# tlk00/BitMagic

Measured on NVIDIA B200. Metric: aggregator input 64Kbit-blocks/s, higher is better.
Workload: dtype u32

## Files before the change

### bitmagic_b200/capi.py

```python
from __future__ import annotations

import ctypes as C
import os
from pathlib import Path

import numpy as np

_HERE = Path(__file__).resolve().parent
LIB_PATH = Path(os.environ.get("BMB200_LIB", str(_HERE / "libbmb200.so")))

OK = 0
ERR_BADALLOC, ERR_BADARG, ERR_RANGE, ERR_RS_IDX_MISSING = 1, 2, 3, 7
ERR_CUDA, ERR_NODEVICE, ERR_UNSUPPORTED = 200, 201, 202
BLOCK_WORDS, BLOCK_BYTES, BLOCK_BITS = 2048, 8192, 65536
GAP_MAX_WORDS, GAP_THRESHOLD, GAP_UNIT_WORDS, SUPERBLOCK = 1280, 1276, 8, 256
BLK_NULL, BLK_FULL, BLK_BIT, BLK_GAP = 0, 1, 2, 3
OP_OR, OP_AND, OP_AND_SUB, OP_XOR, OP_SHIFT_R_AND = 0, 1, 2, 3, 4
F_COUNT_ONLY, F_OPT_NONE, F_OPT_COMPRESS, F_OR_TARGET = 1, 0, 2, 4

SYMBOLS = [
    "bmb200_init", "bmb200_destroy", "bmb200_error_msg", "bmb200_last_error", "bmb200_ctx_set_stream",
    "bmb200_ctx_get_stream", "bmb200_ctx_sync", "bmb200_ctx_launch_count", "bmb200_device_info", "bmb200_ctx_set_tuning",
    "bmb200_set_upload", "bmb200_set_upload_vectors", "bmb200_set_adopt_device", "bmb200_set_info",
    "bmb200_set_column_sizes", "bmb200_set_download", "bmb200_set_device_ptrs", "bmb200_set_free",
    "bmb200_synth_set", "bmb200_aggregate", "bmb200_result_optimize", "bmb200_result_total",
    "bmb200_result_fetch_meta", "bmb200_result_sizes", "bmb200_result_fetch", "bmb200_result_device_ptrs",
    "bmb200_result_free", "bmb200_aggregate_host", "bmb200_rs_build", "bmb200_rs_export", "bmb200_rs_total",
    "bmb200_rank_batch", "bmb200_select_batch", "bmb200_rank_batch_dev", "bmb200_select_batch_dev",
    "bmb200_rs_free", "bmb200_rs_rebuild", "bmb200_aggregate_batch", "bmb200_result_group_totals", "bmb200_result_or_target",
    "bmb200_scan", "bmb200_set_upload_blobs", "bmb200_result_fetch_view", "bmb200_ctx_bind_host_numa",
    "bmb200_shard_range", "bmb200_comm_unique_id", "bmb200_comm_init", "bmb200_comm_info", "bmb200_comm_destroy",
    "bmb200_exchange_popcounts", "bmb200_exchange_fence", "bmb200_exchange_fetch", "bmb200_ctx_trim", "bmb200_binop",
    "bmb200_set_upload_slabs", "bmb200_host_slabs_prefetch", "bmb200_host_slab_alloc", "bmb200_host_slab_free",
    "bmb200_result_fetch_view_async", "bmb200_result_fetch_wait", "bmb200_exchange_mode",
    "bmb200_result_fetch_column",
]
OP_SUB = 5
COMM_ID_BYTES = 128
TUNE_GAP_MODE, TUNE_CTAS_PER_SM, TUNE_HOST_THREADS = 0, 1, 2


class PackedSetC(C.Structure):
    _fields_ = [
        ("n_vec", C.c_uint32), ("n_blocks", C.c_uint32),
        ("desc", C.c_void_p), ("bit_base", C.c_void_p), ("gap_base", C.c_void_p),
        ("bit_pool", C.c_void_p), ("gap_pool", C.c_void_p),
    ]


class VecBlocksC(C.Structure):
    _fields_ = [("n_blocks", C.c_uint32), ("kind", C.c_void_p), ("ptr", C.c_void_p)]


class HostSlabC(C.Structure):
# ... 109 lines not shown
            pass

    def sync(self):
        self.check(lib().bmb200_ctx_sync(self._h), "ctx_sync")

    def set_stream(self, cuda_stream: int):
        self.check(lib().bmb200_ctx_set_stream(self._h, C.c_void_p(int(cuda_stream))), "ctx_set_stream")

    def get_stream(self) -> int:
        s = C.c_void_p(0)
        self.check(lib().bmb200_ctx_get_stream(self._h, C.byref(s)), "ctx_get_stream")
        return int(s.value or 0)

    def set_tuning(self, key: int, value: int):
        self.check(lib().bmb200_ctx_set_tuning(self._h, int(key), int(value)), "ctx_set_tuning")

    def launch_count(self) -> int:
        n = C.c_uint64(0)
        self.check(lib().bmb200_ctx_launch_count(self._h, C.byref(n)), "launch_count")
        return int(n.value)

    def trim(self):
        self.check(lib().bmb200_ctx_trim(self._h), "ctx_trim")

    def bind_host_numa(self) -> int:
        node = C.c_int(-1)
        self.check(lib().bmb200_ctx_bind_host_numa(self._h, C.byref(node)), "ctx_bind_host_numa")
        return node.value

    @staticmethod
# ... 383 lines not shown
```

### bitmagic_b200/csrc/agg_kernel.cuh

```cuda
#pragma once
#include "common.cuh"
#include <type_traits>

namespace bmb200 {

constexpr int kAggThreads = 512;
constexpr int kAggWarps   = kAggThreads / 32;
constexpr int kAggChunk   = 1024;
#ifndef BMB200_AGG_CHUNK_WIDE
#define BMB200_AGG_CHUNK_WIDE 1408
#endif
constexpr int kAggChunkWide = BMB200_AGG_CHUNK_WIDE;

#ifndef BMB200_CTAS_PER_SM
#define BMB200_CTAS_PER_SM 2
#endif
#ifndef BMB200_GAP_STAGES
#define BMB200_GAP_STAGES (BMB200_CTAS_PER_SM >= 3 ? 3 : 4)
#endif
#ifndef BMB200_BIT_UNROLL
#define BMB200_BIT_UNROLL 4
#endif
#ifndef BMB200_GAP_CHUNK
#define BMB200_GAP_CHUNK 16384
#endif
#ifndef BMB200_LANES_PER_BLOCK
#define BMB200_LANES_PER_BLOCK 16
#endif
#ifndef BMB200_VAR_UNROLL2
#define BMB200_VAR_UNROLL2 1
#endif
#ifndef BMB200_VAR_SLEEP_NS
#define BMB200_VAR_SLEEP_NS 64
#endif
constexpr uint32_t kLanesPerBlock = BMB200_LANES_PER_BLOCK;
constexpr uint32_t kGroupsPerWarp = 32u / kLanesPerBlock;
constexpr int      kGapStages     = BMB200_GAP_STAGES;
constexpr uint32_t kGapChunkBytes = BMB200_GAP_CHUNK;
constexpr uint32_t kRingBytes     = kGapStages * kGapChunkBytes;
constexpr int      kCtasPerSm     = BMB200_CTAS_PER_SM;
constexpr int      kBitUnroll     = BMB200_BIT_UNROLL;
constexpr uint32_t kRingWords     = kRingBytes / 4;
constexpr uint32_t kGapMaxBytes   = 2560;
constexpr int      kMaxChunks     = (kAggChunk * 4096) / (int)kGapChunkBytes + 4;
constexpr uint32_t kRingTail      = kGapMaxBytes + 512;
constexpr size_t   kAggRingSmem   = kRingBytes + kRingTail;
constexpr uint32_t kLiveAlign     = 8192u;
__host__ inline size_t agg_dyn_smem(size_t static_bytes, size_t reserved_bytes)
{
// ... 21 lines not shown
    uint32_t  compress;
    uint32_t  store_blocks;
    uint32_t  gap_mode;
    uint32_t  dyn_bytes;
    uint32_t  binary;
    uint64_t  gap_pool_bytes;
    uint32_t* blocks;
    uint32_t* popcnt;
    uint64_t* digest;
    uint32_t* nruns;
    uint8_t*  kind;
    uint16_t* gaps;
    unsigned long long* total;
    uint32_t* or_blocks;
    uint32_t* work_counter;
};

constexpr uint32_t kFlNull0 = 1u;
constexpr uint32_t kFlFull0 = 2u;
constexpr uint32_t kFlFull1 = 4u;
constexpr uint32_t kRelMask = BMB200_DESC_REL_MASK;
constexpr uint32_t kEntFlat = BMB200_DESC_GAP_FLAT >> 2;
constexpr uint32_t kFlatMinBlocks = 16u;

__device__ __forceinline__ uint32_t smem_u32(const void* p) { return (uint32_t)__cvta_generic_to_shared(p); }
__device__ __forceinline__ void mbar_init(uint64_t* bar, uint32_t count)
{
    asm volatile("mbarrier.init.shared::cta.b64 [%0], %1;" :: "r"(smem_u32(bar)), "r"(count) : "memory");
}
__device__ __forceinline__ void mbar_arrive_expect_tx(uint64_t* bar, uint32_t bytes)
// ... 24 lines not shown
}
__device__ __forceinline__ uint32_t atoms_add(uint32_t a, uint32_t v)
{
    uint32_t old; asm volatile("atom.shared.add.u32 %0, [%1], %2;" : "=r"(old) : "r"(a), "r"(v) : "memory"); return old;
}
__device__ __forceinline__ void sts32(uint32_t a, uint32_t v) { asm volatile("st.shared.u32 [%0], %1;" :: "r"(a), "r"(v) : "memory"); }
__device__ __forceinline__ void bulk_g2s(void* smem_dst, const void* gsrc, uint32_t bytes, uint64_t* bar)
{
    asm volatile("cp.async.bulk.shared::cluster.global.mbarrier::complete_tx::bytes [%0], [%1], %2, [%3];"
                 :: "r"(smem_u32(smem_dst)), "l"(gsrc), "r"(bytes), "r"(smem_u32(bar)) : "memory");
}
__device__ __forceinline__ void fence_proxy_async()
{
    asm volatile("fence.proxy.async.shared::cta;" ::: "memory");
}

__device__ __forceinline__ uint32_t lds32(uint32_t a) { uint32_t v; asm volatile("ld.shared.u32 %0, [%1];" : "=r"(v) : "r"(a)); return v; }
__device__ __forceinline__ uint32_t lds16(uint32_t a) { uint16_t v; asm volatile("ld.shared.u16 %0, [%1];" : "=h"(v) : "r"(a)); return (uint32_t)v; }
__device__ __forceinline__ uint4 lds128(uint32_t a)
{
    uint4 v; asm volatile("ld.shared.v4.u32 {%0,%1,%2,%3}, [%4];" : "=r"(v.x), "=r"(v.y), "=r"(v.z), "=r"(v.w) : "r"(a)); return v;
}
__device__ __forceinline__ void reds_and(uint32_t a, uint32_t v) { asm volatile("red.shared.and.b32 [%0], %1;" :: "r"(a), "r"(v) : "memory"); }
__device__ __forceinline__ void reds_xor(uint32_t a, uint32_t v) { asm volatile("red.shared.xor.b32 [%0], %1;" :: "r"(a), "r"(v) : "memory"); }
__device__ __forceinline__ uint32_t bmsk(uint32_t pos, uint32_t width)
{
    uint32_t m; asm("bmsk.clamp.b32 %0, %1, %2;" : "=r"(m) : "r"(pos), "r"(width)); return m;
}

template <int OP>
__device__ __forceinline__ void acc_apply0(uint4& a, const uint4& v)
{
    if (OP == BMB200_OP_OR)       { a.x |= v.x; a.y |= v.y; a.z |= v.z; a.w |= v.w; }
    else if (OP == BMB200_OP_XOR) { a.x ^= v.x; a.y ^= v.y; a.z ^= v.z; a.w ^= v.w; }
    else                          { a.x &= v.x; a.y &= v.y; a.z &= v.z; a.w &= v.w; }
}
__device__ __forceinline__ void acc_or(uint4& a, const uint4& v)
{
    a.x |= v.x; a.y |= v.y; a.z |= v.z; a.w |= v.w;
}

template <int OP, bool ROLE1>
__device__ __forceinline__ void bit_phase(const uint4* __restrict__ seg, const uint32_t* lst, uint32_t n, uint4& acc)
{
    const uint4 ident = (!ROLE1 && (OP == BMB200_OP_AND || OP == BMB200_OP_AND_SUB))
                            ? make_uint4(~0u, ~0u, ~0u, ~0u) : make_uint4(0u, 0u, 0u, 0u);
    for (uint32_t i = 0; i < n; i += kBitUnroll) {
        uint4 v[kBitUnroll];
#pragma unroll
        for (int u = 0; u < kBitUnroll; ++u) {
            if (i + u < n) v[u] = ld_stream_v4(seg + (size_t)lst[i + u] * (kBlockWords / 4));
            else           v[u] = ident;
        }
#pragma unroll
        for (int u = 0; u < kBitUnroll; ++u) {
            if (ROLE1) acc_or(acc, v[u]); else acc_apply0<OP>(acc, v[u]);
        }
    }
}

template <bool XOR>
__device__ __forceinline__ void apply_word(uint32_t a, uint32_t m)
{
    if (XOR) reds_xor(a, m); else reds_and(a, ~m);
}
template <bool XOR>
__device__ __forceinline__ void apply_run(uint32_t Ls, uint32_t s, uint32_t e)
{
    const uint32_t ws = s >> 5, we = e >> 5;
    const uint32_t m0 = 0xffffffffu << (s & 31u);
    const uint32_t m1 = 0xffffffffu >> (31u - (e & 31u));
// ... 273 lines not shown
        if (tid == 0) {
            const uint32_t lvl = runs <= 124u ? 0u : runs <= 252u ? 1u : runs <= 508u ? 2u : 3u;
            gout[runs] = 65535u;
            gout[0] = (uint16_t)((R.x & 1u) | (lvl << 1) | (runs << 3));
        }
    }
    if (tid == 0) {
        p.popcnt[col] = tpc;
        p.digest[col] = dg;
        p.nruns[col]  = runs;
        p.kind[col]   = (uint8_t)kd;
        if (tpc) atomicAdd(p.total + grp, (unsigned long long)tpc);
    }
}

template <int OP>
__global__ void __launch_bounds__(kAggThreads, kCtasPerSm) agg_kernel(const AggParams p)
{
    constexpr int kChunkN = (OP == BMB200_OP_AND_SUB) ? kAggChunk : kAggChunkWide;
    constexpr int kMaxChunksN = (kChunkN * 4096) / (int)kGapChunkBytes + 4;
    extern __shared__ __align__(128) uint8_t dyn_smem[];
    const uint32_t dyn_s = smem_u32(dyn_smem);
    const uint32_t k_off = ((dyn_s + kLiveAlign - 1u) & ~(kLiveAlign - 1u)) - dyn_s;
    if (k_off + kLiveAlign + (uint32_t)kAggRingSmem > p.dyn_bytes) __trap();
    uint32_t* K = reinterpret_cast<uint32_t*>(dyn_smem + k_off);
    uint32_t* ring = reinterpret_cast<uint32_t*>(dyn_smem + k_off + kLiveAlign);

    __shared__ uint32_t lst_bit0[kChunkN];
    __shared__ uint32_t lst_bit1[kChunkN];
    __shared__ uint32_t lst_gap[kChunkN];
    __shared__ uint32_t s_cfirst[kMaxChunksN];
    __shared__ __align__(8) uint64_t s_full[kGapStages];
    __shared__ uint32_t s_done[kGapStages];
    __shared__ __align__(8) uint64_t s_wfull[kAggWarps * kFlatSlots];
    __shared__ uint32_t s_flat_next;
    __shared__ uint2 s_wpk[2][kAggWarps];
    __shared__ uint32_t s_stat[4];
    __shared__ uint32_t s_flat[3];
    __shared__ uint32_t s_col, s_gap_next;
    __shared__ uint32_t s_pc[kAggWarps], s_tr[kAggWarps], s_dg[kAggWarps];

    constexpr bool kIsXor = (OP == BMB200_OP_XOR);
    constexpr bool kIsAnd = (OP == BMB200_OP_AND || OP == BMB200_OP_AND_SUB);
    constexpr int  kFlatList = (OP == BMB200_OP_OR) ? 0 : (OP == BMB200_OP_AND_SUB) ? 1 : -1;

    const int tid = threadIdx.x, lane = tid & 31, warp = tid >> 5;
    const uint32_t M = p.set.n_vec;
    uint4* K4 = reinterpret_cast<uint4*>(K);
    uint32_t Ks, ring_s;
    asm volatile("mov.u32 %0, %1;" : "=r"(Ks) : "r"(smem_u32(K)));
    asm volatile("mov.u32 %0, %1;" : "=r"(ring_s) : "r"(smem_u32(ring)));
    uint32_t done_s, wfull_s, flat_next_s;
    asm volatile("mov.u32 %0, %1;" : "=r"(flat_next_s) : "r"(smem_u32(&s_flat_next)));
    asm volatile("mov.u32 %0, %1;" : "=r"(done_s) : "r"(smem_u32(s_done)));
    asm volatile("mov.u32 %0, %1;" : "=r"(wfull_s) : "r"(smem_u32(&s_wfull[warp * kFlatSlots])));
    uint32_t wphase = 0;
    uint32_t wchunk[kFlatSlots];
    uint32_t gseq = 0;

    if (tid == 0) {
#pragma unroll
        for (int s = 0; s < kGapStages; ++s) mbar_init(&s_full[s], 1u);
#pragma unroll
        for (int w = 0; w < kAggWarps * (int)kFlatSlots; ++w) mbar_init(&s_wfull[w], 1u);
        asm volatile("fence.mbarrier_init.release.cluster;" ::: "memory");
    }
    uint32_t next_item = 0;
    if (tid == 0) next_item = atomicAdd(p.work_counter, 1u);
    __syncthreads();

    for (;;) {
        if (tid == 0) s_col = next_item;
        __syncthreads();
        const uint32_t item = s_col;
        if (item >= p.n_cols * p.n_groups) break;
        if (tid == 0) next_item = atomicAdd(p.work_counter, 1u);
        const uint32_t colx = item / p.n_groups, grp = item - colx * p.n_groups;
        const uint32_t col = grp * p.n_cols + colx;
        const uint32_t nb = p.nb_from + colx;
        const uint32_t gb0 = p.goff[2u * grp], gb1 = p.goff[2u * grp + 1u], gb2 = p.goff[2u * grp + 2u];
        const uint32_t n0 = gb1 - gb0, n1 = (OP == BMB200_OP_AND_SUB) ? gb2 - gb1 : 0u;
        const uint32_t ntot = n0 + n1;
        const uint32_t* gmem = p.group + gb0;
        uint32_t rule = 0u;
        if (p.binary) {
            const uint32_t* dr = p.set.desc + (size_t)nb * M;
            rule = binop_rule(p.binary - 1u, dr[gmem[0]] & 3u, dr[gmem[1]] & 3u);
            if (rule & kRuleMerge) {
                if (p.kind[col] != 0xffu) { __syncthreads(); continue; }
                rule = kRuleComputed;
// ... 35 lines not shown
                const uint32_t lt = (1u << lane) - 1u;
                const uint32_t m0 = __ballot_sync(0xffffffffu, c0), m1 = __ballot_sync(0xffffffffu, c1);
                const uint32_t m2 = __ballot_sync(0xffffffffu, c2), m3 = __ballot_sync(0xffffffffu, c3);
                if (lane == 0) s_wpk[trip][warp] = make_uint2(__popc(m0) | (__popc(m1) << 16), __popc(m2) | (__popc(m3) << 16));
                __syncthreads();
                uint2 x = (lane < kAggWarps) ? s_wpk[trip][lane] : make_uint2(0u, 0u);
#pragma unroll
                for (int o = 1; o < kAggWarps; o <<= 1) {
                    const uint32_t y0 = __shfl_up_sync(0xffffffffu, x.x, o), y1 = __shfl_up_sync(0xffffffffu, x.y, o);
                    if (lane >= o) { x.x += y0; x.y += y1; }
                }
                const uint32_t t01 = __shfl_sync(0xffffffffu, x.x, kAggWarps - 1), t23 = __shfl_sync(0xffffffffu, x.y, kAggWarps - 1);
                uint32_t e01 = __shfl_sync(0xffffffffu, x.x, (warp + 31) & 31), e23 = __shfl_sync(0xffffffffu, x.y, (warp + 31) & 31);
                if (warp == 0) { e01 = 0u; e23 = 0u; }
                e01 += run01; e23 += run23;
                if (c0) lst_bit0[(e01 & 0xffffu) + __popc(m0 & lt)] = rel;
                if (c1) lst_bit1[(e01 >> 16) + __popc(m1 & lt)] = rel;
                if (c2) lst_gap[(e23 & 0xffffu) + __popc(m2 & lt)] = rel;
                if (c3) lst_gap[kChunkN - 1 - ((e23 >> 16) + __popc(m3 & lt))] = rel;
                run01 += t01; run23 += t23;
            }
            fl = __reduce_or_sync(0xffffffffu, fl);
            nfull0 = warp_sum(nfull0);
            nonflat = __reduce_or_sync(0xffffffffu, nonflat);
            if (lane == 0) { if (fl) atomicOr(&s_stat[0], fl); if (nfull0) atomicAdd(&s_stat[3], nfull0); if (nonflat) s_flat[2] = 1u; }
            const uint32_t nbit0 = run01 & 0xffffu, nbit1 = run01 >> 16, ngap0 = run23 & 0xffffu, ngap1 = run23 >> 16;
            if (tid == 0) { s_stat[1] += nbit0; s_stat[2] += ngap0; }
            __syncthreads();

            const uint32_t want0 = kIsAnd ? 0u : 1u;
            bool ok0 = false, ok1 = false;
            bool flat = false;
// ... 44 lines not shown
            auto issue_fill = [&](uint32_t wlo, uint32_t wbytes, uint32_t c, bool mirror) {
                const uint32_t s = (gseq + c) % kGapStages;
                const uint32_t off = c * kGapChunkBytes;
                const uint32_t bytes = min(kGapChunkBytes, wbytes - off);
                const uint32_t extra = (s || !mirror) ? 0u : min(kGapMaxBytes, bytes);
                const uint8_t* src = reinterpret_cast<const uint8_t*>(gseg) + (size_t)wlo * 16u + off;
                mbar_arrive_expect_tx(&s_full[s], bytes + extra);
                bulk_g2s(reinterpret_cast<uint8_t*>(ring) + s * kGapChunkBytes, src, bytes, &s_full[s]);
                if (extra) bulk_g2s(reinterpret_cast<uint8_t*>(ring) + kRingBytes, src, extra, &s_full[s]);
            };
            auto flat_big = [&](uint32_t wbytes) -> bool {
                return BMB200_FLAT_SLOTS == 1 ? true : BMB200_FLAT_SLOTS == 2 ? false : wbytes >= (uint32_t)BMB200_FLAT_BIG_WINDOW;
            };
            auto flat_claim = [&](auto S) -> uint32_t {
                uint32_t c = 0;
                if (lane == 0) c = atoms_add(flat_next_s, 1u) * decltype(S)::value;
                return __shfl_sync(0xffffffffu, c, 0);
            };
            auto flat_fill = [&](auto S, uint32_t wlo, uint32_t wbytes, uint32_t c, uint32_t k) {
                constexpr uint32_t kChunk = kFlatWarpBytes / decltype(S)::value;
                if (lane == 0) {
                    const uint32_t off = c * kChunk;
                    const uint32_t bytes = min(kChunk, wbytes - off);
                    const uint32_t bar = wfull_s + 8u * k;
                    fence_proxy_async();
                    asm volatile("mbarrier.arrive.expect_tx.shared::cta.b64 _, [%0], %1;" :: "r"(bar), "r"(bytes) : "memory");
                    asm volatile("cp.async.bulk.shared::cluster.global.mbarrier::complete_tx::bytes [%0], [%1], %2, [%3];"
                                 :: "r"(ring_s + (uint32_t)warp * kFlatWarpBytes + k * kChunk),
                                    "l"(reinterpret_cast<const uint8_t*>(gseg) + (size_t)wlo * 16u + off), "r"(bytes), "r"(bar) : "memory");
                }
            };
// ... 98 lines not shown
                const uint32_t n = q ? ngap1 : ngap0;
                for (;;) {
                    uint32_t g = 0;
                    if (lane == 0) g = atomicAdd(&s_gap_next, 1u);
                    g = __shfl_sync(0xffffffffu, g, 0);
                    if (g >= n) break;
                    const uint32_t ent = q ? lst_gap[kChunkN - 1 - g] : lst_gap[g];
                    gap_scatter_gather<kIsXor>(Ks, gseg + (size_t)(ent & kRelMask) * kGapUnit + (ent >> 29), want, lane);
                }
            };

            const bool flat0 = flat && kFlatList == 0, flat1 = flat && kFlatList == 1;
            const bool str0 = ok0 || flat0, str1 = ok1 || flat1;
            const int first_q = flat ? kFlatList : (ok0 ? 0 : (ok1 ? 1 : -1));
            if (first_q >= 0) stream_setup(first_q, flat);

            bit_phase<OP, false>(bseg, lst_bit0, nbit0, acc0);
            if (OP == BMB200_OP_AND_SUB) bit_phase<OP, true>(bseg, lst_bit1, nbit1, acc1);
            {
                uint4 l = K4[tid];
                if (kIsXor)      { l.x ^= acc0.x; l.y ^= acc0.y; l.z ^= acc0.z; l.w ^= acc0.w; acc0 = make_uint4(0u, 0u, 0u, 0u); }
                else if (kIsAnd) { l.x &= acc0.x & ~acc1.x; l.y &= acc0.y & ~acc1.y; l.z &= acc0.z & ~acc1.z; l.w &= acc0.w & ~acc1.w; }
                else             { l.x &= ~acc0.x; l.y &= ~acc0.y; l.z &= ~acc0.z; l.w &= ~acc0.w; }
                K4[tid] = l;
            }
            __syncthreads();

            if (flat) {
                const uint32_t n = kFlatList ? ngap1 : ngap0;
                for (uint32_t i = tid; i < n; i += kAggThreads) {
                    const uint32_t ent = kFlatList ? lst_gap[kChunkN - 1 - i] : lst_gap[i];
                    if (!(ent >> 29)) apply_run<false>(Ks, 0u, gseg[(size_t)(ent & kRelMask) * kGapUnit + 1u]);
                }
                flat_consume(kFlatList);
            } else if (first_q >= 0) stream_consume(first_q, first_q ? 1u : want0);
            {
                const int second_q = (first_q == 0 && str1) ? 1 : (first_q == 1 && str0 ? 0 : -1);
                if (second_q >= 0) {
                    __syncthreads();
                    stream_setup(second_q, false);
                    stream_consume(second_q, second_q ? 1u : want0);
                }
            }
            if (ngap0 && !str0) gather_pass(0, want0);
            if (ngap1 && !str1) {
                if (ngap0 && !str0) { __syncthreads(); if (tid == 0) s_gap_next = 0u; __syncthreads(); }
                gather_pass(1, 1u);
            }
            __syncthreads();
        }

        const uint32_t flags = s_stat[0], tot_bit0 = s_stat[1], tot_gap0 = s_stat[2], tot_full0 = s_stat[3];
        const uint4 k4 = K4[tid];
        uint4 R;
        int state;
        if (OP == BMB200_OP_OR) {
            if (flags & kFlFull0) state = 1;
            else if (tot_bit0 + tot_gap0 == 0) state = 0;
            else {
                state = 2;
                const int ones = __syncthreads_and((acc0.x & acc0.y & acc0.z & acc0.w) == 0xffffffffu);
                if (ones && tot_bit0 >= 2) state = 1;
            }
            R = make_uint4(~k4.x, ~k4.y, ~k4.z, ~k4.w);
// ... 1 lines not shown
            state = (tot_bit0 + tot_gap0 + tot_full0) ? 2 : 0;
            const uint32_t inv = (tot_full0 & 1u) ? 0xffffffffu : 0u;
            R = make_uint4(k4.x ^ inv, k4.y ^ inv, k4.z ^ inv, k4.w ^ inv);
        } else {
            if ((flags & kFlNull0) || n0 == 0) state = 0;
            else if (flags & kFlFull1) state = 0;
            else if (tot_bit0 + tot_gap0 == 0 && (OP == BMB200_OP_AND || n1 == 0)) state = 1;
            else state = 2;
            R = k4;
        }
        if (state == 0) R = make_uint4(0u, 0u, 0u, 0u);
        if (state == 1) R = make_uint4(~0u, ~0u, ~0u, ~0u);

        finish_block<OP != BMB200_OP_OR>(p, col, colx, grp, R, state, K, s_pc, s_tr, s_dg, rule);
    }
}


__global__ void __launch_bounds__(kAggThreads, kCtasPerSm) finalize_blocks_kernel(const AggParams p, const uint32_t* __restrict__ src)
{
    __shared__ __align__(16) uint32_t K[kBlockWords];
    __shared__ uint32_t s_pc[kAggWarps], s_tr[kAggWarps], s_dg[kAggWarps];
    for (uint32_t col = blockIdx.x; col < p.n_cols; col += gridDim.x) {
        const uint4 R = reinterpret_cast<const uint4*>(src)[(size_t)col * (kBlockWords / 4) + threadIdx.x];
        finish_block<true>(p, col, col, 0u, R, 2, K, s_pc, s_tr, s_dg);
        __syncthreads();
    }
}

}
// ... 1 lines not shown
```

### bitmagic_b200/csrc/capi.cu

```cuda
#include <cstdio>
#include <cstdlib>
#include <cstring>
#include <new>
#include <string>
#include <vector>

#include "agg_kernel.cuh"
#include "aux_kernels.cuh"
#include "scan_kernel.cuh"
#include "shift_kernel.cuh"
#include "binop_kernel.cuh"
#include <algorithm>
#include <chrono>
#include <cstdio>
#include <cstdlib>
#include "blob_kernel.cuh"
#include "blob_entropy.cuh"
#include "host_pack.hpp"
#include "comm.hpp"
#include "xchg_kernel.cuh"
#include <sched.h>
#include <fstream>

using namespace bmb200;
// ... 8 lines not shown
    size_t hbm_bytes = 0;
    uint32_t* d_work = nullptr;
    uint32_t* d_group = nullptr;
    size_t group_cap = 0;
    uint32_t* h_group = nullptr;
    std::vector<uint32_t> last_group;
    int agg_ctas_per_sm = kCtasPerSm;
    bmb200_set* host_set = nullptr;
    bmb200_result* host_res = nullptr;
    size_t cap_desc = 0, cap_base = 0, cap_bit = 0, cap_gap = 0;
    uint8_t* h_stage = nullptr;
    size_t h_stage_cap = 0;
    void* d_tmp[13] = {};
    size_t d_tmp_cap[13] = {};
    int gap_mode = 0;
    bool attr_set = false, merge_attr_set = false;
    size_t agg_dyn[4] = {};
    int host_threads = 0;
    uint8_t* h_ring[kStageSlots] = {};
    size_t h_ring_cap = 0;
    cudaEvent_t ring_ev[kStageSlots] = {};
    void* d_pool[8] = {};
    size_t d_pool_cap[8] = {};
    std::vector<std::pair<uint64_t, uint64_t>> mirror_sig;
    bool mirror_live = false;
    void* h_pool[8] = {};
    size_t h_pool_cap[8] = {};
    cudaEvent_t fetch_ev[8] = {};
    unsigned fetch_flip = 0;
    CommState comm;
// ... 240 lines not shown
    ctx->sm_count = prop.multiProcessorCount;
    ctx->cc_major = prop.major; ctx->cc_minor = prop.minor;
    ctx->hbm_bytes = prop.totalGlobalMem;
    if (cudaSetDevice(device) != cudaSuccess ||
        cudaStreamCreateWithFlags(&ctx->stream, cudaStreamNonBlocking) != cudaSuccess ||
        cudaMalloc((void**)&ctx->d_work, 64) != cudaSuccess) {
        delete ctx; return BMB200_ERR_CUDA;
    }
    ctx->own_stream = true;
    const char* e = getenv("BMB200_AGG_CTAS_PER_SM");
    if (e) bmb200_ctx_set_tuning(ctx, BMB200_TUNE_CTAS_PER_SM, atoi(e));
    e = getenv("BMB200_GAP_MODE");
    if (e) bmb200_ctx_set_tuning(ctx, BMB200_TUNE_GAP_MODE, atoi(e));
    e = getenv("BMB200_HOST_THREADS");
    if (e) bmb200_ctx_set_tuning(ctx, BMB200_TUNE_HOST_THREADS, atoi(e));
    *out = ctx;
    return BMB200_OK;
}

int bmb200_destroy(bmb200_ctx* ctx)
{
    if (!ctx) return BMB200_ERR_BADARG;
    cudaSetDevice(ctx->device);
    cudaStreamSynchronize(ctx->stream);
    if (ctx->host_res) bmb200_result_free(ctx->host_res);
    if (ctx->host_set) bmb200_set_free(ctx->host_set);
    bmb200_ctx_trim(ctx);
    if (ctx->own_stream) cudaStreamDestroy(ctx->stream);
    cudaFree(ctx->d_work); cudaFree(ctx->d_group);
    if (ctx->h_group) cudaFreeHost(ctx->h_group);
// ... 51 lines not shown
{
    if (!ctx) return BMB200_ERR_BADARG;
    if (sm_count) *sm_count = ctx->sm_count;
    if (cc_major) *cc_major = ctx->cc_major;
    if (cc_minor) *cc_minor = ctx->cc_minor;
    if (hbm_bytes) *hbm_bytes = ctx->hbm_bytes;
    return BMB200_OK;
}

int bmb200_ctx_set_tuning(bmb200_ctx* ctx, int key, int value)
{
    if (!ctx) return BMB200_ERR_BADARG;
    if (key == BMB200_TUNE_GAP_MODE && (value == 0 || value == 1)) { ctx->gap_mode = value; return BMB200_OK; }
    if (key == BMB200_TUNE_CTAS_PER_SM && value >= 1 && value <= kCtasPerSm) { ctx->agg_ctas_per_sm = value; return BMB200_OK; }
    if (key == BMB200_TUNE_HOST_THREADS && value >= 0 && value <= 64) { ctx->host_threads = value; return BMB200_OK; }
    return BMB200_ERR_BADARG;
}


static int set_alloc(bmb200_ctx* ctx, uint32_t n_vec, uint32_t n_blocks, uint64_t n_bit, uint64_t n_gap_units,
                     bmb200_set** out)
{
    bmb200_set* s = new (std::nothrow) bmb200_set();
    if (!s) return BMB200_ERR_BADALLOC;
    s->ctx = ctx; s->owns = true;
    s->v.n_vec = n_vec; s->v.n_blocks = n_blocks;
    s->n_bit_blocks = n_bit; s->n_gap_units = n_gap_units;
    s->gap_pool_bytes = n_gap_units * 16ull + kSlack;
    int rc;
    uint32_t* desc = nullptr; uint64_t *bb = nullptr, *gb = nullptr; uint32_t* bp = nullptr; uint16_t* gp = nullptr;
// ... 659 lines not shown
    return BMB200_OK;
}

int bmb200_ctx_trim(bmb200_ctx* ctx)
{
    if (!ctx) return BMB200_ERR_BADARG;
    cudaSetDevice(ctx->device);
    cudaStreamSynchronize(ctx->stream);
    auto& a = ctx->arena;
    if (a.full) { cudaFree(a.desc); cudaFree(a.bb); cudaFree(a.gb); cudaFree(a.bp); cudaFree(a.gp); a = bmb200_ctx::Arena(); }
    for (int slot = 6; slot <= 7; ++slot)
        if (ctx->d_pool[slot]) { cudaFree(ctx->d_pool[slot]); ctx->d_pool[slot] = nullptr; ctx->d_pool_cap[slot] = 0; }
    return BMB200_OK;
}

int bmb200_synth_set(bmb200_ctx* ctx, uint32_t n_vec, uint32_t n_blocks,
                     const double* density, const uint64_t* seed, int optimize, bmb200_set** out)
{
    if (!ctx || !out || !density || !seed || !n_vec || !n_blocks) return BMB200_ERR_BADARG;
    if ((uint64_t)n_vec * n_blocks > 0x7fffffffull) return BMB200_ERR_RANGE;
    CU(cudaSetDevice(ctx->device));
    cudaStream_t st = ctx->stream;
    std::vector<uint32_t> thr(n_vec);
    for (uint32_t v = 0; v < n_vec; ++v) {
        double t = density[v] * 65536.0 + 0.5;
        thr[v] = t <= 0 ? 0u : t >= 65536.0 ? 65536u : (uint32_t)t;
    }
    const size_t items = (size_t)n_vec * n_blocks;
    uint64_t* d_seed = nullptr; uint32_t* d_thr = nullptr; uint8_t* d_kind = nullptr; uint16_t* d_glen = nullptr;
    uint64_t *d_cb = nullptr, *d_cg = nullptr;
// ... 164 lines not shown
        if (ce == cudaSuccess && or_target) ce = cudaMemsetAsync(r->or_blocks, 0, (size_t)cols * BMB200_BLOCK_BYTES, ctx->stream);
        if (ce != cudaSuccess) {
            ctx->last_err = std::string("aggregate: ") + cudaGetErrorString(ce);
            if (!*inout) bmb200_result_free(r);
            return BMB200_ERR_CUDA;
        }
        if (!same) { try { ctx->last_group.assign(ctx->h_group, ctx->h_group + nwords); } catch (...) { ctx->last_group.clear(); } }
    }

    AggParams p{};
    p.set = set->v; p.group = ctx->d_group; p.goff = ctx->d_group + nmem; p.n_groups = ng;
    p.nb_from = a->nb_from; p.n_cols = cols;
    p.compress = compress ? 1u : 0u; p.store_blocks = store ? 1u : 0u;
    p.blocks = r->blocks; p.popcnt = r->popcnt; p.digest = r->digest; p.nruns = r->nruns; p.kind = r->kind; p.gaps = r->gaps;
    p.total = r->total; p.work_counter = ctx->d_work; p.or_blocks = or_target ? r->or_blocks : nullptr;
    p.gap_mode = (uint32_t)ctx->gap_mode; p.gap_pool_bytes = set->gap_pool_bytes;
    cudaError_t ae = cudaSuccess; set_agg_attrs(ctx, &ae);
    if (ae != cudaSuccess) { ctx->last_err = std::string("cudaFuncSetAttribute: ") + cudaGetErrorString(ae); if (!*inout) bmb200_result_free(r); return BMB200_ERR_CUDA; }
    uint32_t grid = (uint32_t)(ctx->sm_count * ctx->agg_ctas_per_sm);
    if (ctx->comm.comm && ctx->comm.nranks > 1 && ctx->sm_count > 8) {
        static const int reserve = []() { const char* e = getenv("BMB200_AGG_RESERVE_SMS"); return e ? atoi(e) : 0; }();
        if (reserve > 0 && reserve < ctx->sm_count) grid = (uint32_t)((ctx->sm_count - reserve) * ctx->agg_ctas_per_sm);
    }
    if (grid > n_cols) grid = n_cols;
    if (a->op != BMB200_OP_SHIFT_R_AND) p.dyn_bytes = (uint32_t)ctx->agg_dyn[a->op];
    switch (a->op) {
    case BMB200_OP_OR:      agg_kernel<BMB200_OP_OR><<<grid, kAggThreads, ctx->agg_dyn[BMB200_OP_OR], ctx->stream>>>(p); break;
    case BMB200_OP_AND:     agg_kernel<BMB200_OP_AND><<<grid, kAggThreads, ctx->agg_dyn[BMB200_OP_AND], ctx->stream>>>(p); break;
    case BMB200_OP_AND_SUB: agg_kernel<BMB200_OP_AND_SUB><<<grid, kAggThreads, ctx->agg_dyn[BMB200_OP_AND_SUB], ctx->stream>>>(p); break;
    case BMB200_OP_SHIFT_R_AND: shift_and_kernel<<<grid, kAggThreads, 0, ctx->stream>>>(p); break;
    default:                agg_kernel<BMB200_OP_XOR><<<grid, kAggThreads, ctx->agg_dyn[BMB200_OP_XOR], ctx->stream>>>(p); break;
// ... 55 lines not shown
    if (e == cudaSuccess && !ctx->merge_attr_set) { e = cudaFuncSetAttribute(gap_merge_kernel, cudaFuncAttributeMaxDynamicSharedMemorySize, (int)kMergeSmem); ctx->merge_attr_set = (e == cudaSuccess); }
    if (e != cudaSuccess) { ctx->last_err = std::string("binop: ") + cudaGetErrorString(e); return bail(BMB200_ERR_CUDA); }
    const uint32_t bop = op == BMB200_OP_OR ? BINOP_OR : op == BMB200_OP_AND ? BINOP_AND : op == BMB200_OP_XOR ? BINOP_XOR : BINOP_SUB;
    MergeParams mp{};
    mp.set = set->v; mp.va = va; mp.vb = vb; mp.op = bop; mp.nb_from = nb_from; mp.n_cols = cols;
    mp.kind = r->kind; mp.popcnt = r->popcnt; mp.digest = r->digest; mp.nruns = r->nruns; mp.gaps = r->gaps; mp.total = r->total;
    uint32_t mgrid = (cols + kMergeWarps - 1) / kMergeWarps; const uint32_t mmax = (uint32_t)ctx->sm_count * 8u; if (mgrid > mmax) mgrid = mmax;
    gap_merge_kernel<<<mgrid, kMergeWarps * 32, kMergeSmem, ctx->stream>>>(mp);
    int rc = after_launch(ctx);
    if (rc) return bail(rc);
    AggParams p{};
    p.set = set->v; p.group = ctx->d_group; p.goff = ctx->d_group + 2; p.n_groups = 1;
    p.nb_from = nb_from; p.n_cols = cols; p.compress = compress ? 1u : 0u; p.store_blocks = 1u;
    p.blocks = r->blocks; p.popcnt = r->popcnt; p.digest = r->digest; p.nruns = r->nruns; p.kind = r->kind; p.gaps = r->gaps;
    p.total = r->total; p.work_counter = ctx->d_work; p.or_blocks = nullptr;
    p.gap_mode = (uint32_t)ctx->gap_mode; p.gap_pool_bytes = set->gap_pool_bytes; p.binary = 1u + bop;
    uint32_t grid = (uint32_t)(ctx->sm_count * ctx->agg_ctas_per_sm); if (grid > cols) grid = cols;
    const int kop = op == BMB200_OP_SUB ? BMB200_OP_AND_SUB : op;
    p.dyn_bytes = (uint32_t)ctx->agg_dyn[kop];
    switch (kop) {
    case BMB200_OP_OR:      agg_kernel<BMB200_OP_OR><<<grid, kAggThreads, ctx->agg_dyn[BMB200_OP_OR], ctx->stream>>>(p); break;
    case BMB200_OP_AND:     agg_kernel<BMB200_OP_AND><<<grid, kAggThreads, ctx->agg_dyn[BMB200_OP_AND], ctx->stream>>>(p); break;
    case BMB200_OP_AND_SUB: agg_kernel<BMB200_OP_AND_SUB><<<grid, kAggThreads, ctx->agg_dyn[BMB200_OP_AND_SUB], ctx->stream>>>(p); break;
    default:                agg_kernel<BMB200_OP_XOR><<<grid, kAggThreads, ctx->agg_dyn[BMB200_OP_XOR], ctx->stream>>>(p); break;
    }
    if ((rc = after_launch(ctx))) return bail(rc);
    *inout = r;
    return BMB200_OK;
}

int bmb200_scan(bmb200_ctx* ctx, const bmb200_set* set, const bmb200_scan_args* a, bmb200_result** inout)
// ... 716 lines not shown
```

### include/bmb200.h

```cpp
#ifndef BMB200_H_INCLUDED
#define BMB200_H_INCLUDED

#include <stddef.h>
#include <stdint.h>

#ifdef __cplusplus
extern "C" {
#endif

#define BMB200_OK                  0
#define BMB200_ERR_BADALLOC        1
#define BMB200_ERR_BADARG          2
#define BMB200_ERR_RANGE           3
#define BMB200_ERR_RS_IDX_MISSING  7
#define BMB200_ERR_CUDA            200
#define BMB200_ERR_NODEVICE        201
#define BMB200_ERR_UNSUPPORTED     202

#define BMB200_BLOCK_WORDS     2048u
#define BMB200_BLOCK_BYTES     8192u
#define BMB200_BLOCK_BITS      65536u
#define BMB200_GAP_MAX_WORDS   1280u
#define BMB200_GAP_THRESHOLD   1276u
#define BMB200_GAP_UNIT_WORDS  8u
// ... 69 lines not shown
    uint32_t* nruns;
} bmb200_result_meta;

int bmb200_init(int device, bmb200_ctx** out);
int bmb200_destroy(bmb200_ctx* ctx);
const char* bmb200_error_msg(int code);
int bmb200_last_error(const bmb200_ctx* ctx, char* buf, size_t buflen);
int bmb200_ctx_set_stream(bmb200_ctx* ctx, void* cuda_stream);
int bmb200_ctx_get_stream(const bmb200_ctx* ctx, void** cuda_stream);
int bmb200_ctx_sync(bmb200_ctx* ctx);
int bmb200_ctx_launch_count(const bmb200_ctx* ctx, uint64_t* out);
int bmb200_device_info(const bmb200_ctx* ctx, int* sm_count, int* cc_major, int* cc_minor, uint64_t* hbm_bytes);
#define BMB200_TUNE_GAP_MODE     0
#define BMB200_TUNE_CTAS_PER_SM  1
#define BMB200_TUNE_HOST_THREADS 2
int bmb200_ctx_set_tuning(bmb200_ctx* ctx, int key, int value);
int bmb200_ctx_bind_host_numa(bmb200_ctx* ctx, int* node);
int bmb200_ctx_trim(bmb200_ctx* ctx);

int bmb200_set_upload(bmb200_ctx* ctx, const bmb200_packed_set* host, bmb200_set** out);
int bmb200_set_upload_vectors(bmb200_ctx* ctx, uint32_t n_vec, uint32_t n_blocks,
                              const bmb200_vec_blocks* vecs, bmb200_set** out);
typedef struct bmb200_host_slab {
    const void* base;
    uint64_t    bytes;
} bmb200_host_slab;
int bmb200_set_upload_slabs(bmb200_ctx* ctx, uint32_t n_vec, uint32_t n_blocks, const bmb200_vec_blocks* vecs,
                            const bmb200_host_slab* slabs, uint32_t n_slabs, bmb200_set** out);
int bmb200_host_slabs_prefetch(bmb200_ctx* ctx, const bmb200_host_slab* slabs, uint32_t n_slabs);
int bmb200_host_slab_alloc(uint64_t bytes, void** out);
int bmb200_host_slab_free(void* slab);
// ... 90 lines not shown
```

Baseline: 7.195 billion.

## Merge AND_SUB bit lists into one streamed loop, unroll 8, add optional L2 prefetch

The two bit-block lists for AND_SUB now share one shared array, filled from opposite ends, and are consumed in a single fused loop instead of two sequential passes. The bit-phase unroll rises from 4 to 8 for more loads in flight. An optional L2 bulk prefetch of the next column's bit pool and descriptors and phase-clock instrumentation are also added, but both are off by default. The fused loop adds a per-element branch, and the larger unroll raises register pressure at 2 CTAs per SM.

```diff
diff --git a/bitmagic_b200/capi.py b/bitmagic_b200/capi.py
--- a/bitmagic_b200/capi.py
+++ b/bitmagic_b200/capi.py
@@ -33,11 +33,12 @@
     "bmb200_exchange_popcounts", "bmb200_exchange_fence", "bmb200_exchange_fetch", "bmb200_ctx_trim", "bmb200_binop",
     "bmb200_set_upload_slabs", "bmb200_host_slabs_prefetch", "bmb200_host_slab_alloc", "bmb200_host_slab_free",
     "bmb200_result_fetch_view_async", "bmb200_result_fetch_wait", "bmb200_exchange_mode",
-    "bmb200_result_fetch_column",
+    "bmb200_result_fetch_column", "bmb200_debug_agg_phases",
 ]
 OP_SUB = 5
 COMM_ID_BYTES = 128
-TUNE_GAP_MODE, TUNE_CTAS_PER_SM, TUNE_HOST_THREADS = 0, 1, 2
+TUNE_GAP_MODE, TUNE_CTAS_PER_SM, TUNE_HOST_THREADS, TUNE_AGG_PREFETCH = 0, 1, 2, 3
+PHASE_ROWS, PHASE_COLS = 1024, 8
 
 
 class PackedSetC(C.Structure):
@@ -177,6 +178,11 @@
 
     def set_tuning(self, key: int, value: int):
         self.check(lib().bmb200_ctx_set_tuning(self._h, int(key), int(value)), "ctx_set_tuning")
+
+    def debug_agg_phases(self) -> np.ndarray:
+        out = np.zeros((PHASE_ROWS, PHASE_COLS), np.uint64)
+        self.check(lib().bmb200_debug_agg_phases(self._h, ptr(out), int(out.size)), "debug_agg_phases")
+        return out
 
     def launch_count(self) -> int:
         n = C.c_uint64(0)
diff --git a/bitmagic_b200/csrc/agg_kernel.cuh b/bitmagic_b200/csrc/agg_kernel.cuh
--- a/bitmagic_b200/csrc/agg_kernel.cuh
+++ b/bitmagic_b200/csrc/agg_kernel.cuh
@@ -19,7 +19,7 @@
 #define BMB200_GAP_STAGES (BMB200_CTAS_PER_SM >= 3 ? 3 : 4)
 #endif
 #ifndef BMB200_BIT_UNROLL
-#define BMB200_BIT_UNROLL 4
+#define BMB200_BIT_UNROLL 8
 #endif
 #ifndef BMB200_GAP_CHUNK
 #define BMB200_GAP_CHUNK 16384
@@ -33,6 +33,10 @@
 #ifndef BMB200_VAR_SLEEP_NS
 #define BMB200_VAR_SLEEP_NS 64
 #endif
+#ifndef BMB200_AGG_L2_PREFETCH
+#define BMB200_AGG_L2_PREFETCH 0
+#endif
+constexpr bool     kAggL2Prefetch = BMB200_AGG_L2_PREFETCH != 0;
 constexpr uint32_t kLanesPerBlock = BMB200_LANES_PER_BLOCK;
 constexpr uint32_t kGroupsPerWarp = 32u / kLanesPerBlock;
 constexpr int      kGapStages     = BMB200_GAP_STAGES;
@@ -84,6 +88,7 @@
     unsigned long long* total;
     uint32_t* or_blocks;
     uint32_t* work_counter;
+    uint32_t  pf_cap;
 };
 
 constexpr uint32_t kFlNull0 = 1u;
@@ -138,6 +143,22 @@
 {
     asm volatile("fence.proxy.async.shared::cta;" ::: "memory");
 }
+__device__ __forceinline__ void prefetch_l2(const void* g, uint32_t bytes)
+{
+    asm volatile("cp.async.bulk.prefetch.L2.global [%0], %1;" :: "l"(g), "r"(bytes) : "memory");
+}
+
+#ifndef BMB200_AGG_PHASE_CLOCKS
+#define BMB200_AGG_PHASE_CLOCKS 0
+#endif
+constexpr int kPhaseRows = 1024, kPhaseCols = 8;
+#if BMB200_AGG_PHASE_CLOCKS
+__device__ unsigned long long g_agg_phase[kPhaseRows * kPhaseCols];
+__device__ __forceinline__ unsigned long long globaltimer_ns()
+{
+    unsigned long long t; asm volatile("mov.u64 %0, %globaltimer;" : "=l"(t)); return t;
+}
+#endif
 
 __device__ __forceinline__ uint32_t lds32(uint32_t a) { uint32_t v; asm volatile("ld.shared.u32 %0, [%1];" : "=r"(v) : "r"(a)); return v; }
 __device__ __forceinline__ uint32_t lds16(uint32_t a) { uint16_t v; asm volatile("ld.shared.u16 %0, [%1];" : "=h"(v) : "r"(a)); return (uint32_t)v; }
@@ -164,11 +185,10 @@
     a.x |= v.x; a.y |= v.y; a.z |= v.z; a.w |= v.w;
 }
 
-template <int OP, bool ROLE1>
+template <int OP>
 __device__ __forceinline__ void bit_phase(const uint4* __restrict__ seg, const uint32_t* lst, uint32_t n, uint4& acc)
 {
-    const uint4 ident = (!ROLE1 && (OP == BMB200_OP_AND || OP == BMB200_OP_AND_SUB))
-                            ? make_uint4(~0u, ~0u, ~0u, ~0u) : make_uint4(0u, 0u, 0u, 0u);
+    const uint4 ident = (OP == BMB200_OP_AND || OP == BMB200_OP_AND_SUB) ? make_uint4(~0u, ~0u, ~0u, ~0u) : make_uint4(0u, 0u, 0u, 0u);
     for (uint32_t i = 0; i < n; i += kBitUnroll) {
         uint4 v[kBitUnroll];
 #pragma unroll
@@ -177,8 +197,25 @@
             else           v[u] = ident;
         }
 #pragma unroll
+        for (int u = 0; u < kBitUnroll; ++u) acc_apply0<OP>(acc, v[u]);
+    }
+}
+template <int N>
+__device__ __forceinline__ void bit_phase_and_sub(const uint4* __restrict__ seg, const uint32_t* lst, uint32_t n0, uint32_t n1,
+                                                  uint4& acc0, uint4& acc1)
+{
+    const uint32_t n = n0 + n1;
+    for (uint32_t i = 0; i < n; i += kBitUnroll) {
+        uint4 v[kBitUnroll];
+#pragma unroll
         for (int u = 0; u < kBitUnroll; ++u) {
-            if (ROLE1) acc_or(acc, v[u]); else acc_apply0<OP>(acc, v[u]);
+            const uint32_t k = i + u;
+            if (k < n) v[u] = ld_stream_v4(seg + (size_t)lst[k < n0 ? k : (uint32_t)N - 1u + n0 - k] * (kBlockWords / 4));
+            else       v[u] = make_uint4(0u, 0u, 0u, 0u);
+        }
+#pragma unroll
+        for (int u = 0; u < kBitUnroll; ++u) {
+            if (i + u < n0) acc_apply0<BMB200_OP_AND_SUB>(acc0, v[u]); else acc_or(acc1, v[u]);
         }
     }
 }
@@ -482,6 +519,12 @@
     }
 }
 
+#if BMB200_AGG_PHASE_CLOCKS
+#define AGG_PHASE_MARK(k) do { if (tid == 0) { const unsigned long long t_ = clock64(); s_clk[k] += t_ - s_clk_last; s_clk_last = t_; } } while (0)
+#else
+#define AGG_PHASE_MARK(k) do { } while (0)
+#endif
+
 template <int OP>
 __global__ void __launch_bounds__(kAggThreads, kCtasPerSm) agg_kernel(const AggParams p)
 {
@@ -494,8 +537,7 @@
     uint32_t* K = reinterpret_cast<uint32_t*>(dyn_smem + k_off);
     uint32_t* ring = reinterpret_cast<uint32_t*>(dyn_smem + k_off + kLiveAlign);
 
-    __shared__ uint32_t lst_bit0[kChunkN];
-    __shared__ uint32_t lst_bit1[kChunkN];
+    __shared__ uint32_t lst_bit[kChunkN];
     __shared__ uint32_t lst_gap[kChunkN];
     __shared__ uint32_t s_cfirst[kMaxChunksN];
     __shared__ __align__(8) uint64_t s_full[kGapStages];
@@ -507,6 +549,11 @@
     __shared__ uint32_t s_flat[3];
     __shared__ uint32_t s_col, s_gap_next;
     __shared__ uint32_t s_pc[kAggWarps], s_tr[kAggWarps], s_dg[kAggWarps];
+    __shared__ const uint8_t* s_pf_src;
+    __shared__ uint32_t s_pf_bytes, s_pf_piece;
+#if BMB200_AGG_PHASE_CLOCKS
+    __shared__ unsigned long long s_clk[5], s_clk_last, s_clk0;
+#endif
 
     constexpr bool kIsXor = (OP == BMB200_OP_XOR);
     constexpr bool kIsAnd = (OP == BMB200_OP_AND || OP == BMB200_OP_AND_SUB);
@@ -532,6 +579,11 @@
 #pragma unroll
         for (int w = 0; w < kAggWarps * (int)kFlatSlots; ++w) mbar_init(&s_wfull[w], 1u);
         asm volatile("fence.mbarrier_init.release.cluster;" ::: "memory");
+#if BMB200_AGG_PHASE_CLOCKS
+        for (int k = 0; k < 5; ++k) s_clk[k] = 0ull;
+        s_clk0 = s_clk_last = clock64();
+        if (blockIdx.x < (unsigned)kPhaseRows) g_agg_phase[blockIdx.x * kPhaseCols + 5] = globaltimer_ns();
+#endif
     }
     uint32_t next_item = 0;
     if (tid == 0) next_item = atomicAdd(p.work_counter, 1u);
@@ -541,7 +593,11 @@
         if (tid == 0) s_col = next_item;
         __syncthreads();
         const uint32_t item = s_col;
+        AGG_PHASE_MARK(3);
         if (item >= p.n_cols * p.n_groups) break;
+#if BMB200_AGG_PHASE_CLOCKS
+        if (tid == 0) ++s_clk[4];
+#endif
         if (tid == 0) next_item = atomicAdd(p.work_counter, 1u);
         const uint32_t colx = item / p.n_groups, grp = item - colx * p.n_groups;
         const uint32_t col = grp * p.n_cols + colx;
@@ -607,8 +663,8 @@
                 uint32_t e01 = __shfl_sync(0xffffffffu, x.x, (warp + 31) & 31), e23 = __shfl_sync(0xffffffffu, x.y, (warp + 31) & 31);
                 if (warp == 0) { e01 = 0u; e23 = 0u; }
                 e01 += run01; e23 += run23;
-                if (c0) lst_bit0[(e01 & 0xffffu) + __popc(m0 & lt)] = rel;
-                if (c1) lst_bit1[(e01 >> 16) + __popc(m1 & lt)] = rel;
+                if (c0) lst_bit[(e01 & 0xffffu) + __popc(m0 & lt)] = rel;
+                if (c1) lst_bit[kChunkN - 1 - ((e01 >> 16) + __popc(m1 & lt))] = rel;
                 if (c2) lst_gap[(e23 & 0xffffu) + __popc(m2 & lt)] = rel;
                 if (c3) lst_gap[kChunkN - 1 - ((e23 >> 16) + __popc(m3 & lt))] = rel;
                 run01 += t01; run23 += t23;
@@ -683,7 +739,14 @@
             };
             auto flat_claim = [&](auto S) -> uint32_t {
                 uint32_t c = 0;
-                if (lane == 0) c = atoms_add(flat_next_s, 1u) * decltype(S)::value;
+                if (lane == 0) {
+                    const uint32_t j = atoms_add(flat_next_s, 1u);
+                    c = j * decltype(S)::value;
+                    if (kAggL2Prefetch && p.pf_cap && j >= (uint32_t)kAggWarps) {
+                        const uint32_t bytes = s_pf_bytes, off = (j - (uint32_t)kAggWarps) * s_pf_piece;
+                        if (off < bytes) prefetch_l2(s_pf_src + off, min(s_pf_piece, bytes - off));
+                    }
+                }
                 return __shfl_sync(0xffffffffu, c, 0);
             };
             auto flat_fill = [&](auto S, uint32_t wlo, uint32_t wbytes, uint32_t c, uint32_t k) {
@@ -812,9 +875,31 @@
             const bool str0 = ok0 || flat0, str1 = ok1 || flat1;
             const int first_q = flat ? kFlatList : (ok0 ? 0 : (ok1 ? 1 : -1));
             if (first_q >= 0) stream_setup(first_q, flat);
-
-            bit_phase<OP, false>(bseg, lst_bit0, nbit0, acc0);
-            if (OP == BMB200_OP_AND_SUB) bit_phase<OP, true>(bseg, lst_bit1, nbit1, acc1);
+            AGG_PHASE_MARK(0);
+
+            bool pf_plan = false;
+            uint64_t pf_b0 = 0, pf_b1 = 0;
+            if (kAggL2Prefetch && p.pf_cap && flat && cs == 0u && tid == 0) {
+                const uint32_t nx = next_item / p.n_groups, gx = next_item - nx * p.n_groups;
+                if (next_item < p.n_cols * p.n_groups && nx != colx) {
+                    const uint32_t nn = p.goff[2u * gx + (OP == BMB200_OP_AND_SUB ? 2u : 1u)] - p.goff[2u * gx];
+                    if (2u * nn >= M) { pf_plan = true; pf_b0 = p.set.bit_base[p.nb_from + nx]; pf_b1 = p.set.bit_base[p.nb_from + nx + 1u]; }
+                }
+            }
+
+            if (OP == BMB200_OP_AND_SUB) bit_phase_and_sub<kChunkN>(bseg, lst_bit, nbit0, nbit1, acc0, acc1);
+            else                         bit_phase<OP>(bseg, lst_bit, nbit0, acc0);
+            if (kAggL2Prefetch && p.pf_cap && tid == 0) {
+                uint32_t bytes = 0;
+                if (pf_plan) {
+                    const uint64_t seg = (pf_b1 - pf_b0) * (uint64_t)BMB200_BLOCK_BYTES;
+                    bytes = (uint32_t)min(seg, (uint64_t)p.pf_cap);
+                    const uint32_t nclaims = ((kFlatList ? wb1 : wb0) + kFlatWarpBytes - 1u) / kFlatWarpBytes;
+                    s_pf_src = reinterpret_cast<const uint8_t*>(p.set.bit_pool) + pf_b0 * (uint64_t)BMB200_BLOCK_BYTES;
+                    s_pf_piece = ((bytes + nclaims - 1u) / nclaims + 15u) & ~15u;
+                }
+                s_pf_bytes = bytes;
+            }
             {
                 uint4 l = K4[tid];
                 if (kIsXor)      { l.x ^= acc0.x; l.y ^= acc0.y; l.z ^= acc0.z; l.w ^= acc0.w; acc0 = make_uint4(0u, 0u, 0u, 0u); }
@@ -823,6 +908,7 @@
                 K4[tid] = l;
             }
             __syncthreads();
+            AGG_PHASE_MARK(1);
 
             if (flat) {
                 const uint32_t n = kFlatList ? ngap1 : ngap0;
@@ -846,6 +932,15 @@
                 gather_pass(1, 1u);
             }
             __syncthreads();
+            AGG_PHASE_MARK(2);
+        }
+        if (kAggL2Prefetch && p.pf_cap && tid == 0) {
+            const uint32_t nx = next_item / p.n_groups;
+            if (next_item < p.n_cols * p.n_groups && nx != colx) {
+                const uint64_t a = reinterpret_cast<uint64_t>(p.set.desc + (size_t)(p.nb_from + nx) * M);
+                const uint64_t lo = (a + 15u) & ~15ull, hi = (a + 4ull * M) & ~15ull;
+                if (hi > lo) prefetch_l2(reinterpret_cast<const void*>(lo), (uint32_t)(hi - lo));
+            }
         }
 
         const uint32_t flags = s_stat[0], tot_bit0 = s_stat[1], tot_gap0 = s_stat[2], tot_full0 = s_stat[3];
@@ -877,6 +972,14 @@
 
         finish_block<OP != BMB200_OP_OR>(p, col, colx, grp, R, state, K, s_pc, s_tr, s_dg, rule);
     }
+#if BMB200_AGG_PHASE_CLOCKS
+    if (tid == 0 && blockIdx.x < (unsigned)kPhaseRows) {
+        unsigned long long* g = g_agg_phase + blockIdx.x * kPhaseCols;
+        for (int k = 0; k < 5; ++k) g[k] += s_clk[k];
+        g[6] = globaltimer_ns();
+        g[7] = clock64() - s_clk0;
+    }
+#endif
 }
 
 
diff --git a/bitmagic_b200/csrc/capi.cu b/bitmagic_b200/csrc/capi.cu
--- a/bitmagic_b200/csrc/capi.cu
+++ b/bitmagic_b200/csrc/capi.cu
@@ -46,6 +46,7 @@
     void* d_tmp[13] = {};
     size_t d_tmp_cap[13] = {};
     int gap_mode = 0;
+    int agg_prefetch = 0;
     bool attr_set = false, merge_attr_set = false;
     size_t agg_dyn[4] = {};
     int host_threads = 0;
@@ -316,6 +317,8 @@
     if (e) bmb200_ctx_set_tuning(ctx, BMB200_TUNE_GAP_MODE, atoi(e));
     e = getenv("BMB200_HOST_THREADS");
     if (e) bmb200_ctx_set_tuning(ctx, BMB200_TUNE_HOST_THREADS, atoi(e));
+    e = getenv("BMB200_AGG_PREFETCH");
+    if (e) bmb200_ctx_set_tuning(ctx, BMB200_TUNE_AGG_PREFETCH, atoi(e));
     *out = ctx;
     return BMB200_OK;
 }
@@ -397,6 +400,10 @@
     if (key == BMB200_TUNE_GAP_MODE && (value == 0 || value == 1)) { ctx->gap_mode = value; return BMB200_OK; }
     if (key == BMB200_TUNE_CTAS_PER_SM && value >= 1 && value <= kCtasPerSm) { ctx->agg_ctas_per_sm = value; return BMB200_OK; }
     if (key == BMB200_TUNE_HOST_THREADS && value >= 0 && value <= 64) { ctx->host_threads = value; return BMB200_OK; }
+    if (key == BMB200_TUNE_AGG_PREFETCH && value >= 0 && value <= (64 << 20)) {
+        if (value && !kAggL2Prefetch) return BMB200_ERR_UNSUPPORTED;
+        ctx->agg_prefetch = value & ~15; return BMB200_OK;
+    }
     return BMB200_ERR_BADARG;
 }
 
@@ -1086,6 +1093,24 @@
     return BMB200_OK;
 }
 
+int bmb200_debug_agg_phases(bmb200_ctx* ctx, uint64_t* out, int n)
+{
+#if BMB200_AGG_PHASE_CLOCKS
+    if (!ctx || !out || n < 0) return BMB200_ERR_BADARG;
+    CU(cudaSetDevice(ctx->device));
+    CU(cudaStreamSynchronize(ctx->stream));
+    const int words = std::min(n, kPhaseRows * kPhaseCols);
+    CU(cudaMemcpyFromSymbol(out, g_agg_phase, (size_t)words * 8));
+    void* d = nullptr;
+    CU(cudaGetSymbolAddress(&d, g_agg_phase));
+    CU(cudaMemset(d, 0, sizeof(unsigned long long) * kPhaseRows * kPhaseCols));
+    return BMB200_OK;
+#else
+    (void)ctx; (void)out; (void)n;
+    return BMB200_ERR_UNSUPPORTED;
+#endif
+}
+
 int bmb200_synth_set(bmb200_ctx* ctx, uint32_t n_vec, uint32_t n_blocks,
                      const double* density, const uint64_t* seed, int optimize, bmb200_set** out)
 {
@@ -1280,7 +1305,7 @@
     p.compress = compress ? 1u : 0u; p.store_blocks = store ? 1u : 0u;
     p.blocks = r->blocks; p.popcnt = r->popcnt; p.digest = r->digest; p.nruns = r->nruns; p.kind = r->kind; p.gaps = r->gaps;
     p.total = r->total; p.work_counter = ctx->d_work; p.or_blocks = or_target ? r->or_blocks : nullptr;
-    p.gap_mode = (uint32_t)ctx->gap_mode; p.gap_pool_bytes = set->gap_pool_bytes;
+    p.gap_mode = (uint32_t)ctx->gap_mode; p.gap_pool_bytes = set->gap_pool_bytes; p.pf_cap = (uint32_t)ctx->agg_prefetch;
     cudaError_t ae = cudaSuccess; set_agg_attrs(ctx, &ae);
     if (ae != cudaSuccess) { ctx->last_err = std::string("cudaFuncSetAttribute: ") + cudaGetErrorString(ae); if (!*inout) bmb200_result_free(r); return BMB200_ERR_CUDA; }
     uint32_t grid = (uint32_t)(ctx->sm_count * ctx->agg_ctas_per_sm);
@@ -1366,7 +1391,7 @@
     p.nb_from = nb_from; p.n_cols = cols; p.compress = compress ? 1u : 0u; p.store_blocks = 1u;
     p.blocks = r->blocks; p.popcnt = r->popcnt; p.digest = r->digest; p.nruns = r->nruns; p.kind = r->kind; p.gaps = r->gaps;
     p.total = r->total; p.work_counter = ctx->d_work; p.or_blocks = nullptr;
-    p.gap_mode = (uint32_t)ctx->gap_mode; p.gap_pool_bytes = set->gap_pool_bytes; p.binary = 1u + bop;
+    p.gap_mode = (uint32_t)ctx->gap_mode; p.gap_pool_bytes = set->gap_pool_bytes; p.binary = 1u + bop; p.pf_cap = (uint32_t)ctx->agg_prefetch;
     uint32_t grid = (uint32_t)(ctx->sm_count * ctx->agg_ctas_per_sm); if (grid > cols) grid = cols;
     const int kop = op == BMB200_OP_SUB ? BMB200_OP_AND_SUB : op;
     p.dyn_bytes = (uint32_t)ctx->agg_dyn[kop];
diff --git a/include/bmb200.h b/include/bmb200.h
--- a/include/bmb200.h
+++ b/include/bmb200.h
@@ -107,7 +107,9 @@
 #define BMB200_TUNE_GAP_MODE     0
 #define BMB200_TUNE_CTAS_PER_SM  1
 #define BMB200_TUNE_HOST_THREADS 2
+#define BMB200_TUNE_AGG_PREFETCH 3
 int bmb200_ctx_set_tuning(bmb200_ctx* ctx, int key, int value);
+int bmb200_debug_agg_phases(bmb200_ctx* ctx, uint64_t* out, int n);
 int bmb200_ctx_bind_host_numa(bmb200_ctx* ctx, int* node);
 int bmb200_ctx_trim(bmb200_ctx* ctx);
 
```

Measured after the change: 6.827 billion, median of 6. -5.1%, worse.
